# thomashirtz/samplers

Measured on AMD Instinct MI355X. Metric: posterior samples/sec (batch×steps/s), DPS CelebA-HQ-256 @1/2/4/8 GPU, higher is better.
Workload: dtype f32

## Files before the change

### include/samplers_hip.h

```cpp
#ifndef SAMPLERS_HIP_H
#define SAMPLERS_HIP_H

#include <stdint.h>

#ifdef __cplusplus
extern "C" {
#endif

typedef void* sp_stream_t;

enum {
    SP_OK = 0,
    SP_EINVAL = -1,
    SP_ELAUNCH = -2,
    SP_EUNSUPPORTED = -3
};

enum {
    SP_OP_IDENTITY = 0,
    SP_OP_INPAINT = 1,
    SP_OP_BLUR = 2,
    SP_OP_MASK = 3,
    SP_OP_SR = 4,
    SP_OP_PSF = 5,
// ... 157 lines not shown
                          int64_t batch, int64_t y_div, const sp_step_rec* sched,
                          const int32_t* cursor, float* v_out, float* rsq_partial,
                          sp_stream_t stream);
int sp_dps_residual_sched_ws(const sp_op* op, const float* x, const float* eps, const float* y,
                             int64_t batch, int64_t y_div, const sp_step_rec* sched,
                             const int32_t* cursor, float* v_out, float* rsq_partial,
                             float* work, sp_stream_t stream);
int sp_dps_update_sched(const sp_op* op, const float* x, const float* eps, const float* y,
                        const float* v, const float* w, const float* rsq_partial,
                        uint64_t seed, int64_t sample_offset, int64_t batch, int64_t y_div,
                        const sp_step_rec* sched, const int32_t* cursor, float* x_out,
                        sp_stream_t stream);

int sp_conv3x3_supported(int32_t cin, int32_t cout, int32_t height, int32_t width);
int64_t sp_conv3x3_packed_size(int32_t cin, int32_t cout);
int sp_conv3x3_pack(const float* w, int32_t cout, int32_t cin, int32_t input_vjp, float* wp,
                    sp_stream_t stream);
int sp_conv3x3_fwd(const float* x, const float* wp, const float* bias, int64_t n, int32_t cin,
                   int32_t cout, int32_t height, int32_t width, float* y, sp_stream_t stream);
int sp_conv3x3_bwd_input(const float* dy, const float* wp_vjp, int64_t n, int32_t cin,
                         int32_t cout, int32_t height, int32_t width, float* dx,
                         sp_stream_t stream);

int sp_conv3x3_thin_supported(int32_t cin, int32_t cout, int32_t height, int32_t width);
int sp_conv3x3_thin_fwd(const float* x, const float* w, const float* bias, int64_t n,
                        int32_t cin, int32_t cout, int32_t height, int32_t width, float* y,
                        sp_stream_t stream);
int sp_conv3x3_thin_bwd_input(const float* dy, const float* w, int64_t n, int32_t cin,
                              int32_t cout, int32_t height, int32_t width, float* dx,
                              sp_stream_t stream);

int sp_conv3x3_s2_supported(int32_t cin, int32_t cout, int32_t height, int32_t width,
                            int32_t input_vjp);
int sp_upsample2x_supported(int32_t height, int32_t width);
int sp_upsample2x(const float* x, int64_t planes, int32_t height, int32_t width, float* y,
                  sp_stream_t stream);
int sp_upsample2x_vjp(const float* dy, int64_t planes, int32_t height, int32_t width, float* dx,
                      sp_stream_t stream);
int sp_conv3x3_s2_pack(const float* w, int32_t cout, int32_t cin, int32_t input_vjp, float* wp,
                       sp_stream_t stream);
int sp_conv3x3_s2_fwd(const float* x, const float* wp, const float* bias, int64_t n, int32_t cin,
                      int32_t cout, int32_t height, int32_t width, float* y, sp_stream_t stream);
int sp_conv3x3_s2_bwd_input(const float* dy, const float* wp_vjp, int64_t n, int32_t cin,
                            int32_t cout, int32_t height, int32_t width, int32_t accumulate,
                            float* dx, sp_stream_t stream);
int64_t sp_conv3x3_s2_workspace(int64_t n, int32_t cin, int32_t cout, int32_t height, int32_t width,
                                int32_t input_vjp);
int sp_conv3x3_s2_fwd_ws(const float* x, const float* wp, const float* bias, int64_t n, int32_t cin,
                         int32_t cout, int32_t height, int32_t width, float* y, float* ws, int64_t ws_bytes,
                         sp_stream_t stream);
int sp_conv3x3_s2_bwd_input_ws(const float* dy, const float* wp_vjp, int64_t n, int32_t cin,
                               int32_t cout, int32_t height, int32_t width, int32_t accumulate,
                               float* dx, float* ws, int64_t ws_bytes, sp_stream_t stream);

int sp_wino3x3_supported(int32_t cin, int32_t cout, int32_t height, int32_t width);
int64_t sp_wino3x3_packed_size(int32_t cin, int32_t cout);
int sp_wino3x3_pack(const float* w, int32_t cout, int32_t cin, int32_t input_vjp, float* up,
                    sp_stream_t stream);
int sp_wino3x3_fwd(const float* x, const float* up, const float* bias, int64_t n, int32_t cin,
                   int32_t cout, int32_t height, int32_t width, float* y, sp_stream_t stream);
int sp_wino3x3_fwd_res(const float* x, const float* up, const float* bias, const float* res,
                       int64_t n, int32_t cin, int32_t cout, int32_t height, int32_t width,
                       float* y, sp_stream_t stream);
int sp_wino3x3_bwd_input(const float* dy, const float* up_vjp, int64_t n, int32_t cin,
                         int32_t cout, int32_t height, int32_t width, float* dx,
                         sp_stream_t stream);
int64_t sp_wino3x3_workspace(int64_t n, int32_t cin, int32_t cout, int32_t height, int32_t width);
int sp_wino3x3_fwd_ws(const float* x, const float* up, const float* bias, const float* res,
                      int64_t n, int32_t cin, int32_t cout, int32_t height, int32_t width,
                      float* y, float* ws, int64_t ws_bytes, sp_stream_t stream);
int sp_wino3x3_bwd_input_ws(const float* dy, const float* up_vjp, int64_t n, int32_t cin,
                            int32_t cout, int32_t height, int32_t width, float* dx, float* ws,
                            int64_t ws_bytes, sp_stream_t stream);
int sp_wino3x3_up_supported(int32_t cin, int32_t cout, int32_t height, int32_t width);
int sp_wino3x3_fwd_up(const float* x, const float* up, const float* bias, int64_t n, int32_t cin,
                      int32_t cout, int32_t height, int32_t width, float* y, sp_stream_t stream);
int sp_wino3x3_bwd_input_pool(const float* dy, const float* up_vjp, int64_t n, int32_t cin,
                              int32_t cout, int32_t height, int32_t width, float* dx,
                              sp_stream_t stream);

int sp_gemm_x6_supported(int32_t m, int32_t k, int64_t hw);
int64_t sp_gemm_x6_packed_size(int32_t m, int32_t k);
int sp_gemm_x6_pack(const float* w, int32_t m, int32_t k, int32_t trans, float* wp, sp_stream_t stream);
int sp_gemm_x6(const float* x1, int32_t c1, const float* x2, int32_t c2, const float* wp,
               const float* bias, const float* res, int64_t n, int64_t hw, float* y1, int32_t o1,
               float* y2, int32_t o2, sp_stream_t stream);

int sp_linear_x6_supported(int64_t tokens, int32_t k, int32_t m);
int sp_linear_x6(const float* x, const float* wp, const float* bias, const float* res, int64_t tokens,
                 int32_t k, int32_t m, float* y, sp_stream_t stream);

int sp_gemm_x6_layout_supported(int64_t n, int64_t hw, int32_t k, int32_t m);
int sp_gemm_x6_layout(const float* x, const float* wp, const float* bias, const float* res, int64_t n,
                      int64_t hw, int32_t k, int32_t m, int32_t in_tm, int32_t out_tm, float* y,
                      sp_stream_t stream);

int64_t sp_gemm_x6_workspace(int64_t n, int64_t hw, int32_t k, int32_t m);
int sp_gemm_x6_ws(const float* x1, int32_t c1, const float* x2, int32_t c2, const float* wp,
                  const float* bias, const float* res, int64_t n, int64_t hw, float* y1, int32_t o1,
                  float* y2, int32_t o2, float* ws, int64_t ws_bytes, sp_stream_t stream);
int sp_linear_x6_ws(const float* x, const float* wp, const float* bias, const float* res, int64_t tokens,
                    int32_t k, int32_t m, float* y, float* ws, int64_t ws_bytes, sp_stream_t stream);
int sp_gemm_x6_layout_ws(const float* x, const float* wp, const float* bias, const float* res, int64_t n,
                         int64_t hw, int32_t k, int32_t m, int32_t in_tm, int32_t out_tm, float* y, float* ws,
                         int64_t ws_bytes, sp_stream_t stream);

// ... 116 lines not shown
```

### samplers_amd/_hip.py

```python

from __future__ import annotations

import ctypes
import os
from pathlib import Path

import torch

LIB_PATH = Path(__file__).resolve().parent / "lib" / "libsamplers_hip.so"
DEBUG_LIB_PATH = Path(__file__).resolve().parent / "lib" / "debug" / "libsamplers_hip.so"

SP_OP_IDENTITY, SP_OP_INPAINT, SP_OP_BLUR, SP_OP_MASK, SP_OP_SR, SP_OP_PSF = 0, 1, 2, 3, 4, 5
SP_OP_PHASE = 6
HALO_KINDS = (SP_OP_BLUR, SP_OP_PSF)

_ERRORS = {-1: "invalid argument", -2: "kernel launch failed", -3: "unsupported"}


class HipLibraryError(RuntimeError):
    """The HIP library is missing, failed to load, or a call returned an error."""


class SpOp(ctypes.Structure):
    _fields_ = [
# ... 84 lines not shown
    "sp_adamw_step_until": (ctypes.c_int, [_P, _P, _P, _P, _I64, ctypes.POINTER(SpAdamWCoefs), _P,
                                           _P]),
    "sp_pixel_opt_step": (ctypes.c_int, [_OPP, _P, _P, _P, _P, _I64, _I64, _F,
                                         ctypes.POINTER(SpAdamWCoefs), _P, _P, _P]),
    "sp_opt_check": (ctypes.c_int, [_P, _I64, _F, ctypes.c_double, _P, _P, _P]),
    "sp_opt_check_plateau": (ctypes.c_int, [_P, _I64, _F, ctypes.c_double, _I64, _I64, _P, _P, _P,
                                            _P]),
    "sp_conv3x3_supported": (ctypes.c_int, [ctypes.c_int32] * 4),
    "sp_conv3x3_packed_size": (_I64, [ctypes.c_int32, ctypes.c_int32]),
    "sp_conv3x3_pack": (ctypes.c_int, [_P, ctypes.c_int32, ctypes.c_int32, ctypes.c_int32, _P, _P]),
    "sp_conv3x3_fwd": (ctypes.c_int, [_P, _P, _P, _I64, ctypes.c_int32, ctypes.c_int32,
                                      ctypes.c_int32, ctypes.c_int32, _P, _P]),
    "sp_conv3x3_bwd_input": (ctypes.c_int, [_P, _P, _I64, ctypes.c_int32, ctypes.c_int32,
                                            ctypes.c_int32, ctypes.c_int32, _P, _P]),
    "sp_conv3x3_thin_supported": (ctypes.c_int, [ctypes.c_int32] * 4),
    "sp_conv3x3_thin_fwd": (ctypes.c_int, [_P, _P, _P, _I64, ctypes.c_int32, ctypes.c_int32,
                                           ctypes.c_int32, ctypes.c_int32, _P, _P]),
    "sp_conv3x3_thin_bwd_input": (ctypes.c_int, [_P, _P, _I64, ctypes.c_int32, ctypes.c_int32,
                                                 ctypes.c_int32, ctypes.c_int32, _P, _P]),
    "sp_conv3x3_s2_supported": (ctypes.c_int, [ctypes.c_int32] * 5),
    "sp_upsample2x_supported": (ctypes.c_int, [ctypes.c_int32] * 2),
    "sp_upsample2x": (ctypes.c_int, [_P, _I64, ctypes.c_int32, ctypes.c_int32, _P, _P]),
    "sp_upsample2x_vjp": (ctypes.c_int, [_P, _I64, ctypes.c_int32, ctypes.c_int32, _P, _P]),
    "sp_attention_supported": (ctypes.c_int, [_I64, _I64, _I64, ctypes.c_int32]),
    "sp_attention_fwd": (ctypes.c_int, [_P, _P, _P, _I64, _I64, ctypes.c_int32, _F, _P, _P, _P]),
    "sp_attention_bwd": (ctypes.c_int, [_P, _P, _P, _P, _P, _P, _I64, _I64, ctypes.c_int32, _F,
                                        _P, _P, _P, _P, _P]),
    "sp_attention_mh_supported": (ctypes.c_int, [_I64, ctypes.c_int32, _I64, _I64, ctypes.c_int32]),
    "sp_attention6_supported": (ctypes.c_int, [_I64, ctypes.c_int32, _I64, ctypes.c_int32]),
    "sp_attention6_fwd_mh": (ctypes.c_int, [_P, _P, _P, _I64, ctypes.c_int32, _I64, ctypes.c_int32,
                                            ctypes.c_int32, ctypes.c_int32, _F, _P, _P, _P]),
    "sp_attention6_workspace": (_I64, [_I64, ctypes.c_int32, _I64, ctypes.c_int32]),
    "sp_attention6_fwd_ws": (ctypes.c_int, [_P, _P, _P, _I64, ctypes.c_int32, _I64, ctypes.c_int32,
                                            ctypes.c_int32, ctypes.c_int32, _F, _P, _P, _P, _I64, _P]),
    "sp_attention_bf16x6": (ctypes.c_int, [ctypes.c_int32]),
    "sp_attention_bf16x6_enabled": (ctypes.c_int, []),
    "sp_attention_fwd_mh": (ctypes.c_int, [_P, _P, _P, _I64, ctypes.c_int32, _I64, _I64, ctypes.c_int32,
                                           ctypes.c_int32, ctypes.c_int32, _I64, ctypes.c_int32, _F, _P, _P,
                                           _P]),
    "sp_attention_bwd_mh": (ctypes.c_int, [_P, _P, _P, _P, _P, _P, _I64, ctypes.c_int32, _I64, _I64,
                                           ctypes.c_int32, ctypes.c_int32, ctypes.c_int32, _I64,
                                           ctypes.c_int32, _F, _P, _P, _P, _P, _P]),
    "sp_conv3x3_s2_pack": (ctypes.c_int, [_P, ctypes.c_int32, ctypes.c_int32, ctypes.c_int32, _P, _P]),
    "sp_conv3x3_s2_fwd": (ctypes.c_int, [_P, _P, _P, _I64, ctypes.c_int32, ctypes.c_int32,
                                         ctypes.c_int32, ctypes.c_int32, _P, _P]),
    "sp_conv3x3_s2_bwd_input": (ctypes.c_int, [_P, _P, _I64, ctypes.c_int32, ctypes.c_int32,
                                               ctypes.c_int32, ctypes.c_int32, ctypes.c_int32, _P, _P]),
    "sp_conv3x3_s2_workspace": (_I64, [_I64, ctypes.c_int32, ctypes.c_int32, ctypes.c_int32, ctypes.c_int32,
                                       ctypes.c_int32]),
    "sp_conv3x3_s2_fwd_ws": (ctypes.c_int, [_P, _P, _P, _I64, ctypes.c_int32, ctypes.c_int32, ctypes.c_int32,
                                            ctypes.c_int32, _P, _P, _I64, _P]),
    "sp_conv3x3_s2_bwd_input_ws": (ctypes.c_int, [_P, _P, _I64, ctypes.c_int32, ctypes.c_int32, ctypes.c_int32,
                                                  ctypes.c_int32, ctypes.c_int32, _P, _P, _I64, _P]),
    "sp_wino3x3_supported": (ctypes.c_int, [ctypes.c_int32] * 4),
    "sp_gemm_x6_supported": (ctypes.c_int, [ctypes.c_int32, ctypes.c_int32, _I64]),
    "sp_gemm_x6_packed_size": (_I64, [ctypes.c_int32, ctypes.c_int32]),
    "sp_gemm_x6_pack": (ctypes.c_int, [_P, ctypes.c_int32, ctypes.c_int32, ctypes.c_int32, _P, _P]),
    "sp_gemm_x6": (ctypes.c_int, [_P, ctypes.c_int32, _P, ctypes.c_int32, _P, _P, _P, _I64, _I64,
                                  _P, ctypes.c_int32, _P, ctypes.c_int32, _P]),
    "sp_linear_x6_supported": (ctypes.c_int, [_I64, ctypes.c_int32, ctypes.c_int32]),
    "sp_linear_x6": (ctypes.c_int, [_P, _P, _P, _P, _I64, ctypes.c_int32, ctypes.c_int32, _P, _P]),
    "sp_gemm_x6_layout_supported": (ctypes.c_int, [_I64, _I64, ctypes.c_int32, ctypes.c_int32]),
    "sp_gemm_x6_layout": (ctypes.c_int, [_P, _P, _P, _P, _I64, _I64, ctypes.c_int32, ctypes.c_int32,
                                         ctypes.c_int32, ctypes.c_int32, _P, _P]),
    "sp_gemm_x6_workspace": (_I64, [_I64, _I64, ctypes.c_int32, ctypes.c_int32]),
    "sp_gemm_x6_ws": (ctypes.c_int, [_P, ctypes.c_int32, _P, ctypes.c_int32, _P, _P, _P, _I64, _I64,
                                     _P, ctypes.c_int32, _P, ctypes.c_int32, _P, _I64, _P]),
    "sp_linear_x6_ws": (ctypes.c_int, [_P, _P, _P, _P, _I64, ctypes.c_int32, ctypes.c_int32, _P, _P, _I64,
                                       _P]),
    "sp_gemm_x6_layout_ws": (ctypes.c_int, [_P, _P, _P, _P, _I64, _I64, ctypes.c_int32, ctypes.c_int32,
                                            ctypes.c_int32, ctypes.c_int32, _P, _P, _I64, _P]),
    "sp_layernorm_supported": (ctypes.c_int, [_I64, ctypes.c_int32]),
    "sp_layernorm_fwd": (ctypes.c_int, [_P, _P, _P, _I64, ctypes.c_int32, _F, _P, _P, _P, _P]),
    "sp_layernorm_bwd": (ctypes.c_int, [_P, _P, _P, _P, _P, _P, _I64, ctypes.c_int32, _P, _P]),
    "sp_geglu_fwd": (ctypes.c_int, [_P, _I64, ctypes.c_int32, _P, _P]),
    "sp_geglu_bwd": (ctypes.c_int, [_P, _P, _I64, ctypes.c_int32, _P, _P]),
    "sp_softmax_rows_supported": (ctypes.c_int, [_I64, ctypes.c_int32]),
    "sp_softmax_rows": (ctypes.c_int, [_P, _I64, ctypes.c_int32, _P, _P]),
    "sp_softmax_bwd_rows": (ctypes.c_int, [_P, _P, _I64, ctypes.c_int32, _F, _P]),
    "sp_conv1x1_small_supported": (ctypes.c_int, [ctypes.c_int32, ctypes.c_int32, _I64]),
    "sp_conv1x1_small": (ctypes.c_int, [_P, _P, _P, _I64, ctypes.c_int32, ctypes.c_int32, _I64,
                                        ctypes.c_int32, _P, _P]),
    "sp_wino3x3_packed_size": (_I64, [ctypes.c_int32, ctypes.c_int32]),
    "sp_wino3x3_pack": (ctypes.c_int, [_P, ctypes.c_int32, ctypes.c_int32, ctypes.c_int32, _P, _P]),
    "sp_wino3x3_fwd": (ctypes.c_int, [_P, _P, _P, _I64, ctypes.c_int32, ctypes.c_int32,
                                      ctypes.c_int32, ctypes.c_int32, _P, _P]),
    "sp_wino3x3_bwd_input": (ctypes.c_int, [_P, _P, _I64, ctypes.c_int32, ctypes.c_int32,
                                            ctypes.c_int32, ctypes.c_int32, _P, _P]),
    "sp_sched_timestep": (ctypes.c_int, [_P, _P, _P, _P]),
    "sp_sched_advance": (ctypes.c_int, [_P, _P]),
    "sp_dps_residual_sched": (ctypes.c_int, [_OPP, _P, _P, _P, _I64, _I64, _P, _P, _P, _P, _P]),
    "sp_dps_update_sched": (ctypes.c_int, [_OPP, _P, _P, _P, _P, _P, _P, _U64, _I64, _I64, _I64,
                                           _P, _P, _P, _P]),
    "sp_groupnorm_workspace": (_I64, [_I64, ctypes.c_int32, _I64, ctypes.c_int32]),
    "sp_groupnorm_silu_fwd": (ctypes.c_int, [_P, _P, _P, _P, _I64, ctypes.c_int32, _I64,
                                             ctypes.c_int32, _F, ctypes.c_int32, _P, _P, _P, _P,
                                             _P]),
    "sp_groupnorm_silu_bwd": (ctypes.c_int, [_P, _P, _P, _P, _P, _P, _P, _I64, ctypes.c_int32,
                                             _I64, ctypes.c_int32, ctypes.c_int32, _P, _P, _P]),
    "sp_groupnorm_silu_fwd2": (ctypes.c_int, [_P, _P, ctypes.c_int32, _P, _P, _P, _I64,
                                              ctypes.c_int32, _I64, ctypes.c_int32, _F,
                                              ctypes.c_int32, _P, _P, _P, _P, _P, _I64, _P]),
    "sp_groupnorm_silu_bwd2": (ctypes.c_int, [_P, _P, _P, ctypes.c_int32, _P, _P, _P, _P, _P,
                                              _I64, ctypes.c_int32, _I64, ctypes.c_int32,
                                              ctypes.c_int32, _P, _P, _P, _P, _P, _P, _P, _I64,
                                              _P]),
# ... 155 lines not shown
```

### samplers_amd/networks/layers.py

```python

from __future__ import annotations

import torch
import torch.nn.functional as F
from torch import Tensor, nn

from .. import _hip
from ..runtime import batch_invariant_enabled, split_k_enabled


def group_norm_act_torch(x: Tensor, groups: int, weight: Tensor | None, bias: Tensor | None,
                         eps: float, act: bool, chan_bias: Tensor | None = None) -> Tensor:
    if chan_bias is not None:
        x = x + chan_bias[:, :, None, None]
    y = F.group_norm(x, groups, weight, bias, eps)
    return F.silu(y) if act else y


_shape_cache: dict = {}


def _query(fn_name: str, *args: int) -> int:
    key = (fn_name, args)
    v = _shape_cache.get(key)
# ... 256 lines not shown
        return torch.nn.grad.conv2d_input(tuple(x_shape), module.weight, dy, padding=1)
    dx = torch.empty(tuple(x_shape), device=dy.device, dtype=torch.float32)
    if algo == "thin":
        _hip.check(lib.sp_conv3x3_thin_bwd_input(_hip.ptr(dy), _hip.ptr(module.weight.detach().contiguous()),
                                                 n, cin, cout, h, w, _hip.ptr(dx),
                                                 _hip.stream_of(dy)), "sp_conv3x3_thin_bwd_input")
        return dx
    if algo == "wino":
        ws = _wino_workspace(lib, n, cout, cin, h, w, dy.device)
        _hip.check(lib.sp_wino3x3_bwd_input_ws(_hip.ptr(dy), _hip.ptr(tile_pack(module, algo, True)),
                                               n, cin, cout, h, w, _hip.ptr(dx), _hip.ptr(ws),
                                               0 if ws is None else ws.numel() * 4,
                                               _hip.stream_of(dy)), "sp_wino3x3_bwd_input_ws")
        return dx
    _hip.check(lib.sp_conv3x3_bwd_input(_hip.ptr(dy), _hip.ptr(tile_pack(module, algo, True)), n, cin,
                                        cout, h, w, _hip.ptr(dx), _hip.stream_of(dy)),
               "sp_direct_conv3x3_bwd_input")
    return dx


class _Conv3x3Fn(torch.autograd.Function):
    @staticmethod
    def forward(ctx, x, weight, bias, module):
        ctx.module = module
        ctx.has_bias = bias is not None
        ctx.save_for_backward(x if weight.requires_grad else None, weight)
        ctx.x_shape = x.shape
        return conv3x3_forward(module, x)

    @staticmethod
    def backward(ctx, dy):
        x, weight = ctx.saved_tensors
        dx = dw = db = None
        if ctx.needs_input_grad[0]:
            dx = conv3x3_input_vjp(ctx.module, dy, ctx.x_shape)
        if ctx.needs_input_grad[1]:
            dw = torch.nn.grad.conv2d_weight(x, weight.shape, dy.contiguous(), padding=1)
        if ctx.has_bias and ctx.needs_input_grad[2]:
            db = dy.sum(dim=(0, 2, 3))
        return dx, dw, db, None


def tile_pack(module: nn.Conv2d, algo: str, input_vjp: bool) -> Tensor:
    w = module.weight
    key = (w.data_ptr(), w._version, w.device)
    cache = module.__dict__.setdefault("_tile_packs", {})
    if cache.get("key") != key:
        cache.clear()
        cache["key"] = key
    if (algo, input_vjp) not in cache:
        lib = _hip.load_library()
        cout, cin = w.shape[0], w.shape[1]
        wc = w.detach().contiguous()
        size_fn, fn = ((lib.sp_wino3x3_packed_size, lib.sp_wino3x3_pack) if algo == "wino"
                       else (lib.sp_conv3x3_packed_size, lib.sp_conv3x3_pack))
        out = torch.empty(int(size_fn(cin, cout)), device=w.device)
        _hip.check(fn(_hip.ptr(wc), cout, cin, int(input_vjp), _hip.ptr(out), _hip.stream_of(wc)),
                   f"sp_{algo}3x3_pack")
        cache[(algo, input_vjp)] = out
    return cache[(algo, input_vjp)]


class Conv3x3(nn.Conv2d):

    def __init__(self, cin: int, cout: int) -> None:
        super().__init__(cin, cout, 3, padding=1)

    def _pack(self, algo: str, input_vjp: bool) -> Tensor:
        return tile_pack(self, algo, input_vjp)

    def forward(self, x: Tensor) -> Tensor:
        if x.is_cuda and x.dtype == torch.bfloat16:
            from . import bf16
            if bf16.conv_supported(self, x):
                return bf16.conv3x3(self, x)
        if x.is_cuda and x.dtype == torch.float32 and x.dim() == 4:
            lib = _hip.load_library()
            n, cin, h, w = x.shape
            if _conv_algo(lib, cin, self.out_channels, h, w, conv_backend()) is not None:
                return _Conv3x3Fn.apply(x, self.weight, self.bias, self)
        miopen_fallback(x)
        return super().forward(x)



def _upsample2x_call(fn_name: str, src: Tensor, out_shape) -> Tensor:
    lib = _hip.load_library()
    n, c, h, w = (src.shape if fn_name == "sp_upsample2x" else out_shape)
    src = src.contiguous()
    out = torch.empty(tuple(out_shape), device=src.device, dtype=torch.float32)
    _hip.check(getattr(lib, fn_name)(_hip.ptr(src), n * c, h, w, _hip.ptr(out),
                                     _hip.stream_of(src)), fn_name)
    return out


class _Upsample2xFn(torch.autograd.Function):
    @staticmethod
    def forward(ctx, x):
        n, c, h, w = x.shape
        ctx.x_shape = x.shape
        return _upsample2x_call("sp_upsample2x", x, (n, c, 2 * h, 2 * w))

    @staticmethod
    def backward(ctx, dy):
        return _upsample2x_call("sp_upsample2x_vjp", dy, ctx.x_shape)


def _upconv_enabled() -> bool:
    import os

    return os.environ.get("SAMPLERS_AMD_UPCONV", "1").lower() not in ("0", "off", "false")
# ... 49 lines not shown
        return _UpsampleConv3x3Fn.apply(x, module.weight, module.bias, module)
    return module(upsample_nearest2x(x))


def upsample_nearest2x(x: Tensor) -> Tensor:
    if (x.is_cuda and x.dtype == torch.float32 and x.dim() == 4 and x.numel() > 0 and
            _hip.load_library().sp_upsample2x_supported(x.shape[2], x.shape[3])):
        return _Upsample2xFn.apply(x)
    return F.interpolate(x, scale_factor=2.0, mode="nearest")



def _s2_packed(module: nn.Conv2d, input_vjp: bool) -> Tensor:
    w = module.weight
    key = (w.data_ptr(), w._version, w.device)
    cache = module.__dict__.setdefault("_s2_packs", {})
    if cache.get("key") != key:
        cache.clear()
        cache["key"] = key
    if input_vjp not in cache:
        lib = _hip.load_library()
        cout, cin = w.shape[0], w.shape[1]
        wc = w.detach().contiguous()
        out = torch.empty(cin * cout * 9, device=w.device)
        _hip.check(lib.sp_conv3x3_s2_pack(_hip.ptr(wc), cout, cin, int(input_vjp), _hip.ptr(out),
                                          _hip.stream_of(wc)), "sp_conv3x3_s2_pack")
        cache[input_vjp] = out
    return cache[input_vjp]


def downsample_s2_supported(module: nn.Conv2d, x: Tensor) -> bool:
    if not (x.is_cuda and x.dtype == torch.float32 and x.dim() == 4) or conv_backend() == "miopen":
        return False
    lib = _hip.load_library()
    _, cin, h, w = x.shape
    cout = module.out_channels
    return bool(lib.sp_conv3x3_s2_supported(cin, cout, h, w, 0) and
                lib.sp_conv3x3_s2_supported(cin, cout, h, w, 1))


class SkipGrad:

    __slots__ = ("grad", "enabled")

    def __init__(self) -> None:
        self.grad: Tensor | None = None
        self.enabled = True

    def take(self) -> Tensor | None:
        g, self.grad = self.grad, None
        return g


def _s2_workspace(lib, n: int, cin: int, cout: int, h: int, w: int, vjp: int, device) -> tuple[Tensor | None, int]:
    nb = _query("sp_conv3x3_s2_workspace", n, cin, cout, h, w, vjp) if split_k_enabled() else 0
    if nb <= 0:
        return None, 0
    return torch.empty(nb // 4, device=device, dtype=torch.float32), nb


class _ConvS2Fn(torch.autograd.Function):
    @staticmethod
    def forward(ctx, x, weight, bias, module, box=None):
        lib = _hip.load_library()
        x = x.contiguous()
        n, cin, h, w = x.shape
        cout = module.out_channels
        y = torch.empty(n, cout, h // 2, w // 2, device=x.device, dtype=torch.float32)
        ws, nb = _s2_workspace(lib, n, cin, cout, h, w, 0, x.device)
        _hip.check(lib.sp_conv3x3_s2_fwd_ws(_hip.ptr(x), _hip.ptr(_s2_packed(module, False)),
                                            _hip.ptr(bias.contiguous()) if bias is not None else None,
                                            n, cin, cout, h, w, _hip.ptr(y), _hip.ptr(ws), nb, _hip.stream_of(x)),
                   "sp_conv3x3_s2_fwd")
        ctx.module = module
        ctx.box = box
        ctx.x_shape = x.shape
        return y

    @staticmethod
    def backward(ctx, dy):
        dx = None
        if ctx.needs_input_grad[0]:
            lib = _hip.load_library()
            n, cin, h, w = ctx.x_shape
            dx = ctx.box.take() if ctx.box is not None else None
            acc = dx is not None
            if dx is None:
                dx = torch.empty(tuple(ctx.x_shape), device=dy.device, dtype=torch.float32)
            ws, nb = _s2_workspace(lib, n, cin, ctx.module.out_channels, h, w, 1, dy.device)
            _hip.check(lib.sp_conv3x3_s2_bwd_input_ws(_hip.ptr(dy.contiguous()),
                                                      _hip.ptr(_s2_packed(ctx.module, True)),
                                                      n, cin, ctx.module.out_channels, h, w, int(acc),
                                                      _hip.ptr(dx), _hip.ptr(ws), nb, _hip.stream_of(dy)),
                       "sp_conv3x3_s2_bwd_input")
        return dx, None, None, None, None



def strided_full_supported(module: nn.Conv2d, x: Tensor) -> bool:
    if not (x.is_cuda and x.dtype == torch.float32 and x.dim() == 4) or module.weight.requires_grad:
        return False
    backend = conv_backend()
    if backend == "miopen":
        return False
    lib = _hip.load_library()
    _, cin, h, w = x.shape
    cout = module.out_channels
    fwd = _conv_algo(lib, cin, cout, h, w, backend)
    vjp = _conv_algo(lib, cout, cin, h, w, backend)
    ok = ("wino", "direct")
    return h % 2 == 0 and w % 2 == 0 and fwd in ok and vjp in ok


class _ConvS2FullFn(torch.autograd.Function):
    @staticmethod
    def forward(ctx, x, weight, bias, module, phase):
        y = conv3x3_forward(module, x.contiguous())
        ctx.module, ctx.phase, ctx.x_shape = module, phase, x.shape
        return y[:, :, phase::2, phase::2].contiguous()

    @staticmethod
    def backward(ctx, dy):
        dx = None
        if ctx.needs_input_grad[0]:
            n, _, h, w = ctx.x_shape
            dyf = dy.new_zeros((n, ctx.module.out_channels, h, w))
            dyf[:, :, ctx.phase::2, ctx.phase::2] = dy
            dx = conv3x3_input_vjp(ctx.module, dyf, ctx.x_shape)
        return dx, None, None, None, None


def conv3x3_stride2(module: nn.Conv2d, x: Tensor, padding: int) -> Tensor:
    if x.is_cuda and x.dtype == torch.bfloat16:
        from . import bf16
        if bf16.strided_supported(module, x):
            return bf16.conv3x3_stride2(module, x, padding)
    if strided_full_supported(module, x):
        return _ConvS2FullFn.apply(x, module.weight, module.bias, module, 0 if padding else 1)
    miopen_fallback(x)
    return module(x) if padding else module(F.pad(x, (0, 1, 0, 1)))


def downsample_conv(module: nn.Conv2d, x: Tensor, box: SkipGrad | None = None) -> Tensor:
    if x.is_cuda and x.dtype == torch.bfloat16:
        if box is not None:
            box.enabled = False
        return conv3x3_stride2(module, x, padding=0)
# ... 324 lines not shown
```

Measured before the change: 230.8.

## Add polyphase Winograd-style MFMA kernel for stride-2 3x3 conv fwd and input-VJP

Adds a new stride-2 3x3 convolution kernel that splits the stride-2 conv into polyphase components with a Winograd-like input transform. It runs the products on 32x32x2 f32 MFMA, using a software-pipelined 4-deep register ring and LDS staging for the forward path. The Python layer routes stride-2 conv forward and backward-input through it by default when supported and split-K workspace is not in use. It aims to cut the arithmetic and memory traffic of the existing direct stride-2 kernel. The cost is a new weight-packing format and a larger, more complex kernel that is harder to maintain.

```diff
diff --git a/include/samplers_hip.h b/include/samplers_hip.h
--- a/include/samplers_hip.h
+++ b/include/samplers_hip.h
@@ -233,6 +233,16 @@
 int sp_conv3x3_s2_bwd_input_ws(const float* dy, const float* wp_vjp, int64_t n, int32_t cin,
                                int32_t cout, int32_t height, int32_t width, int32_t accumulate,
                                float* dx, float* ws, int64_t ws_bytes, sp_stream_t stream);
+int sp_conv3x3_s2p_supported(int32_t cin, int32_t cout, int32_t height, int32_t width,
+                             int32_t input_vjp);
+int64_t sp_conv3x3_s2p_packed_size(int32_t cin, int32_t cout);
+int sp_conv3x3_s2p_pack(const float* w, int32_t cout, int32_t cin, int32_t input_vjp, float* up,
+                        sp_stream_t stream);
+int sp_conv3x3_s2p_fwd(const float* x, const float* up, const float* bias, int64_t n, int32_t cin,
+                       int32_t cout, int32_t height, int32_t width, float* y, sp_stream_t stream);
+int sp_conv3x3_s2p_bwd_input(const float* dy, const float* up_vjp, int64_t n, int32_t cin,
+                             int32_t cout, int32_t height, int32_t width, int32_t accumulate,
+                             float* dx, sp_stream_t stream);
 
 int sp_wino3x3_supported(int32_t cin, int32_t cout, int32_t height, int32_t width);
 int64_t sp_wino3x3_packed_size(int32_t cin, int32_t cout);
diff --git a/samplers_amd/_hip.py b/samplers_amd/_hip.py
--- a/samplers_amd/_hip.py
+++ b/samplers_amd/_hip.py
@@ -160,6 +160,13 @@
                                             ctypes.c_int32, _P, _P, _I64, _P]),
     "sp_conv3x3_s2_bwd_input_ws": (ctypes.c_int, [_P, _P, _I64, ctypes.c_int32, ctypes.c_int32, ctypes.c_int32,
                                                   ctypes.c_int32, ctypes.c_int32, _P, _P, _I64, _P]),
+    "sp_conv3x3_s2p_supported": (ctypes.c_int, [ctypes.c_int32] * 5),
+    "sp_conv3x3_s2p_packed_size": (_I64, [ctypes.c_int32, ctypes.c_int32]),
+    "sp_conv3x3_s2p_pack": (ctypes.c_int, [_P, ctypes.c_int32, ctypes.c_int32, ctypes.c_int32, _P, _P]),
+    "sp_conv3x3_s2p_fwd": (ctypes.c_int, [_P, _P, _P, _I64, ctypes.c_int32, ctypes.c_int32,
+                                          ctypes.c_int32, ctypes.c_int32, _P, _P]),
+    "sp_conv3x3_s2p_bwd_input": (ctypes.c_int, [_P, _P, _I64, ctypes.c_int32, ctypes.c_int32,
+                                                ctypes.c_int32, ctypes.c_int32, ctypes.c_int32, _P, _P]),
     "sp_wino3x3_supported": (ctypes.c_int, [ctypes.c_int32] * 4),
     "sp_gemm_x6_supported": (ctypes.c_int, [ctypes.c_int32, ctypes.c_int32, _I64]),
     "sp_gemm_x6_packed_size": (_I64, [ctypes.c_int32, ctypes.c_int32]),
diff --git a/samplers_amd/csrc/sp_conv_s2p.hip b/samplers_amd/csrc/sp_conv_s2p.hip
--- /dev/null
+++ b/samplers_amd/csrc/sp_conv_s2p.hip
@@ -0,0 +1,568 @@
+
+#define SP_TU 18
+#include "sp_common.h"
+
+namespace sp {
+
+typedef float p2_f32x16 __attribute__((ext_vector_type(16)));
+typedef float p2_f32x4 __attribute__((ext_vector_type(4)));
+typedef float p2_f32x2 __attribute__((ext_vector_type(2)));
+
+constexpr int P2_M = 64;
+constexpr int P2_OOB = 0x7FFFFFF0;
+constexpr int P2_USLOT = 16 * 64;
+
+struct P2Win { float a[3][3]; float b[2][3]; };
+struct P2U { p2_f32x4 u[4]; };
+
+struct P2Off { int v[8]; };
+
+template <bool VJP> struct P2Raw;
+template <> struct P2Raw<false> { p2_f32x4 a, b; float e; };
+template <> struct P2Raw<true> { p2_f32x2 r[3]; float e[3]; };
+
+template <int TSH> struct P2F {
+    static constexpr int TCW = 1 << TSH, TRW = 32 >> TSH, R = 4 * TRW + 1;
+    static constexpr int PS = TCW + 1, RS = 4 * PS, CS = R * RS;
+    static constexpr int PIECES = 2 * R * TCW;
+};
+constexpr int P2F_STAGE = 1344;
+constexpr int P2F_SINK = 2 * P2F_STAGE;
+constexpr int P2F_LDS = 3 * P2F_STAGE + 512;
+
+template <bool VJP, int S, int WV>
+__device__ __forceinline__ void p2_load(__amdgpu_buffer_rsrc_t rs, const P2Off& o, P2Raw<VJP>& w) {
+    if constexpr (!VJP) {
+        w.a = __builtin_bit_cast(p2_f32x4, __builtin_amdgcn_raw_buffer_load_b128(rs, o.v[0], 0, 0));
+        if constexpr (WV == 1)
+            w.b = __builtin_bit_cast(p2_f32x4, __builtin_amdgcn_raw_buffer_load_b128(rs, o.v[1], 0, 0));
+        if constexpr (WV == 2) w.e = __uint_as_float(__builtin_amdgcn_raw_buffer_load_b32(rs, o.v[2], 0, 0));
+    } else {
+#pragma unroll
+        for (int i = 0; i < 3; ++i)
+            w.r[i] = __builtin_bit_cast(p2_f32x2, __builtin_amdgcn_raw_buffer_load_b64(rs, o.v[i], 0, 0));
+#pragma unroll
+        for (int i = (S ? 1 : 0); i < 3; ++i)
+            w.e[i] = __uint_as_float(__builtin_amdgcn_raw_buffer_load_b32(rs, o.v[3 + i], 0, 0));
+    }
+}
+
+template <int TSH, int WV>
+__device__ __forceinline__ void p2f_stage(float* st, const P2Off& o, const P2Raw<false>& w) {
+    constexpr int PS = P2F<TSH>::PS;
+#pragma unroll
+    for (int q = 0; q < 4; ++q) st[o.v[3] + q * PS] = w.a[q];
+    if constexpr (WV == 1) {
+#pragma unroll
+        for (int q = 0; q < 4; ++q) st[o.v[4] + q * PS] = w.b[q];
+    }
+    if constexpr (WV == 2) st[o.v[5]] = w.e;
+}
+
+template <int S, int TSH>
+__device__ __forceinline__ void p2f_window(const float* st, int rd, P2Win& w) {
+    constexpr int PS = P2F<TSH>::PS, RS = P2F<TSH>::RS;
+    const float* p = st + rd;
+    if constexpr (S == 0) {
+#pragma unroll
+        for (int i = 0; i < 3; ++i)
+            w.a[i][0] = p[2 * i * RS], w.a[i][1] = p[2 * i * RS + 2 * PS], w.a[i][2] = p[2 * i * RS + 1];
+#pragma unroll
+        for (int i = 0; i < 2; ++i)
+            w.b[i][0] = p[(2 * i + 1) * RS + PS], w.b[i][1] = p[(2 * i + 1) * RS + 3 * PS];
+    } else {
+#pragma unroll
+        for (int i = 0; i < 3; ++i) w.a[i][0] = p[2 * i * RS + PS], w.a[i][1] = p[2 * i * RS + 3 * PS];
+#pragma unroll
+        for (int i = 0; i < 2; ++i)
+            w.b[i][0] = p[(2 * i + 1) * RS], w.b[i][1] = p[(2 * i + 1) * RS + 2 * PS],
+            w.b[i][2] = p[(2 * i + 1) * RS + 1];
+    }
+}
+
+template <int S>
+__device__ __forceinline__ void p2_window(const P2Raw<true>& x, P2Win& w) {
+    const auto& r = x.r;
+    const auto& e = x.e;
+    if constexpr (S == 0) {
+#pragma unroll
+        for (int i = 0; i < 3; ++i) w.a[i][0] = e[i], w.a[i][1] = r[i][0], w.a[i][2] = r[i][1];
+#pragma unroll
+        for (int i = 0; i < 2; ++i) w.b[i][0] = r[i + 1][0], w.b[i][1] = r[i + 1][1];
+    } else {
+#pragma unroll
+        for (int i = 0; i < 3; ++i) w.a[i][0] = r[i][0], w.a[i][1] = r[i][1];
+#pragma unroll
+        for (int i = 0; i < 2; ++i) w.b[i][0] = e[i + 1], w.b[i][1] = r[i + 1][0], w.b[i][2] = r[i + 1][1];
+    }
+}
+
+template <int S>
+__device__ __forceinline__ void p2_load_u(__amdgpu_buffer_rsrc_t urs, int lane, int soff, P2U& u) {
+#pragma unroll
+    for (int i = 0; i < 3; ++i)
+        u.u[i] = __builtin_bit_cast(p2_f32x4, __builtin_amdgcn_raw_buffer_load_b128(urs, (i * 64 + lane) * 16, soff, 0));
+    if constexpr (S == 0)
+        u.u[3][0] = __uint_as_float(__builtin_amdgcn_raw_buffer_load_b32(urs, (3 * 64 + lane) * 16, soff, 0));
+}
+
+template <int S>
+__device__ __forceinline__ void p2_transform(const P2Win& w, float (&v)[13]) {
+    if constexpr (S == 0) {
+        float t[3][3];
+#pragma unroll
+        for (int c = 0; c < 3; ++c) {
+            t[0][c] = w.a[0][c] - w.a[1][c];
+            t[1][c] = w.a[1][c];
+            t[2][c] = w.a[2][c] - w.a[1][c];
+        }
+#pragma unroll
+        for (int r = 0; r < 3; ++r) {
+            v[3 * r + 0] = t[r][0] - t[r][1];
+            v[3 * r + 1] = t[r][1];
+            v[3 * r + 2] = t[r][2] - t[r][1];
+        }
+#pragma unroll
+        for (int i = 0; i < 4; ++i) v[9 + i] = w.b[i >> 1][i & 1];
+    } else {
+#pragma unroll
+        for (int c = 0; c < 2; ++c) {
+            v[0 + c] = w.a[0][c] - w.a[1][c];
+            v[2 + c] = w.a[1][c];
+            v[4 + c] = w.a[2][c] - w.a[1][c];
+        }
+#pragma unroll
+        for (int r = 0; r < 2; ++r) {
+            v[6 + 3 * r + 0] = w.b[r][0] - w.b[r][1];
+            v[6 + 3 * r + 1] = w.b[r][1];
+            v[6 + 3 * r + 2] = w.b[r][2] - w.b[r][1];
+        }
+        v[12] = 0.f;
+    }
+}
+
+template <bool VJP> struct P2Ring {
+    P2Raw<VJP> xs[4];
+    P2U us[4];
+    float v[2][13];
+};
+
+#define P2_MFMA(j)                                                                                        \
+    if constexpr ((j) < (S ? 12 : 13)) {                                                                  \
+        acc[j] = __builtin_amdgcn_mfma_f32_32x32x2f32(u.u[(j) >> 2][(j) & 3], vc[j], acc[j], 0, 0, 0);    \
+        __builtin_amdgcn_sched_barrier(0);                                                                \
+    }                                                                                                     \
+    static_assert(true, "")
+#define P2_WALL                    \
+    asm volatile("" ::: "memory"); \
+    __builtin_amdgcn_sched_barrier(0)
+
+template <int S, int U>
+__device__ __forceinline__ void p2_step(const float* __restrict__ inn, int64_t iplane2, int ibytes,
+                                        const P2Off& o, __amdgpu_buffer_rsrc_t urs, int lane, int ustride,
+                                        int q, int nk, P2Ring<true>& r, p2_f32x16 (&acc)[13]) {
+    asm volatile("" : "+s"(q));
+    const P2U& u = r.us[U];
+    const float(&vc)[13] = r.v[U & 1];
+    const int qn = min(q + 3, nk - 1);
+    P2_MFMA(0);
+    {
+        const auto rs = __builtin_amdgcn_make_buffer_rsrc(const_cast<float*>(inn + qn * iplane2), (short)0,
+                                                          ibytes, 0x00020000);
+        p2_load<true, S, S>(rs, o, r.xs[(U + 3) & 3]);
+    }
+    P2_WALL;
+    P2_MFMA(1);
+    p2_load_u<S>(urs, lane, qn * ustride, r.us[(U + 3) & 3]);
+    P2_WALL;
+    P2_MFMA(2);
+    P2_MFMA(3);
+    P2_MFMA(4);
+    P2_MFMA(5);
+    P2_MFMA(6);
+    {
+        P2Win w;
+        p2_window<S>(r.xs[(U + 1) & 3], w);
+        p2_transform<S>(w, r.v[(U + 1) & 1]);
+    }
+    P2_WALL;
+    P2_MFMA(7);
+    P2_MFMA(8);
+    P2_MFMA(9);
+    P2_MFMA(10);
+    P2_MFMA(11);
+    P2_MFMA(12);
+}
+
+template <int WV, int TSH, int U>
+__device__ __forceinline__ void p2f_step(const float* __restrict__ inn, int64_t iplane2, int ibytes,
+                                         const P2Off& o, __amdgpu_buffer_rsrc_t urs, int lane, int ustride,
+                                         int q, int nk, float* xl, P2Ring<false>& r, p2_f32x16 (&acc)[13]) {
+    constexpr int S = WV & 1;
+    asm volatile("" : "+s"(q));
+    const P2U& u = r.us[U];
+    const float(&vc)[13] = r.v[U & 1];
+    P2_MFMA(0);
+    {
+        const auto rs = __builtin_amdgcn_make_buffer_rsrc(
+            const_cast<float*>(inn + min(q + 4, nk - 1) * iplane2), (short)0, ibytes, 0x00020000);
+        p2_load<false, S, WV>(rs, o, r.xs[U]);
+    }
+    P2_WALL;
+    P2_MFMA(1);
+    p2_load_u<S>(urs, lane, min(q + 3, nk - 1) * ustride, r.us[(U + 3) & 3]);
+    P2_WALL;
+    P2_MFMA(2);
+    p2f_stage<TSH, WV>(xl + (U & 1) * P2F_STAGE, o, r.xs[(U + 2) & 3]);
+    P2_WALL;
+    P2_MFMA(3);
+    P2_MFMA(4);
+    P2Win w;
+    p2f_window<S, TSH>(xl + ((U + 1) & 1) * P2F_STAGE, o.v[6], w);
+    P2_WALL;
+    P2_MFMA(5);
+    P2_MFMA(6);
+    P2_MFMA(7);
+    p2_transform<S>(w, r.v[(U + 1) & 1]);
+    P2_WALL;
+    P2_MFMA(8);
+    P2_MFMA(9);
+    P2_MFMA(10);
+    P2_MFMA(11);
+    P2_MFMA(12);
+    __builtin_amdgcn_s_waitcnt(0xc07f);
+    __builtin_amdgcn_s_barrier();
+    P2_WALL;
+}
+#undef P2_MFMA
+#undef P2_WALL
+
+template <bool VJP, int WV, int TSH>
+__device__ __forceinline__ void p2_body(const float* __restrict__ in, const float* __restrict__ up,
+                                        const float* __restrict__ bias, float* __restrict__ out,
+                                        int K, int M, int H, int W, int acc_in, float* ex, float* xl) {
+    constexpr int S = WV & 1;
+    const int Ho = H / 2, Wo = W / 2, TH = Ho / 2, TW = Wo / 2;
+    constexpr int tsh = TSH, tcw = 1 << tsh, trw = 32 >> tsh;
+    const int mblocks = M / P2_M;
+    const int mb = blockIdx.x % mblocks, grp = blockIdx.x / mblocks;
+    const int gw = TW / tcw, per_img = gw * (TH / trw);
+    const int n = grp / per_img, g = grp - n * per_img;
+    const int tid = threadIdx.x, lane = tid & 63, hh = lane >> 5, l = lane & 31;
+    const int wv = __builtin_amdgcn_readfirstlane(tid >> 6);
+    const int ti = (g / gw) * trw + (l >> tsh), tj = (g % gw) * tcw + (l & (tcw - 1));
+    const int m0 = mb * P2_M + (wv >> 1) * 32;
+    SP_DCHECK(TW % tcw == 0 && TH % trw == 0 && ti < TH && tj < TW && m0 + 32 <= M && K % 8 == 0);
+
+    const int ih = VJP ? Ho : H, iw = VJP ? Wo : W;
+    const int64_t iplane = (int64_t)ih * iw;
+    const float* inn = in + (int64_t)n * K * iplane;
+    const int hoff = hh * static_cast<int>(iplane);
+    P2Off o;
+    if constexpr (!VJP) {
+        using F = P2F<TSH>;
+        const int r0 = 4 * (g / gw) * trw, c0 = 4 * (g % gw) * tcw;
+        const int plane = static_cast<int>(iplane);
+#pragma unroll
+        for (int j = 0; j < 2; ++j) {
+            const int it = j ? kBlock + lane : tid;
+            const int c = it / (F::R * tcw), rem = it - c * (F::R * tcw), row = rem >> tsh, c4 = rem & (tcw - 1);
+            const bool have = it < F::PIECES;
+            SP_DCHECK(!have || (c < 2 && row < F::R && c0 + 4 * c4 + 3 < W));
+            o.v[j] = have && r0 + row < H ? (c * plane + (r0 + row) * W + c0 + 4 * c4) * 4 : P2_OOB;
+            o.v[3 + j] = have ? c * F::CS + row * F::RS + c4 : P2F_SINK + tid;
+        }
+        {
+            const int c = lane / F::R, row = lane - c * F::R;
+            const bool have = lane < 2 * F::R;
+            o.v[2] = have && r0 + row < H && c0 + 4 * tcw < W ? (c * plane + (r0 + row) * W + c0 + 4 * tcw) * 4
+                                                              : P2_OOB;
+            o.v[5] = have ? c * F::CS + row * F::RS + tcw : P2F_SINK + tid;
+        }
+        o.v[6] = hh * F::CS + 4 * (l >> tsh) * F::RS + (l & (tcw - 1));
+        static_assert(2 * F::CS <= P2F_STAGE && P2F_SINK + kBlock + 3 * F::PS <= 2 * P2F_STAGE + 512, "LDS stage");
+    } else {
+#pragma unroll
+        for (int i = 0; i < 3; ++i) {
+            const int r = 2 * ti - 1 + i;
+            o.v[i] = r >= 0 ? (hoff + r * Wo + 2 * tj) * 4 : P2_OOB;
+            o.v[3 + i] = (r >= 0 && tj > 0) ? (hoff + r * Wo + 2 * tj - 1) * 4 : P2_OOB;
+        }
+    }
+    const int nk = K / 2;
+    const int ibytes = static_cast<int>(2 * iplane * 4);
+    const int ustride = (M / 32) * 2 * P2_USLOT * 4;
+    const auto urs = __builtin_amdgcn_make_buffer_rsrc(
+        const_cast<float*>(up + ((int64_t)(m0 / 32) * 2 + S) * P2_USLOT), (short)0, 0x7FFFFFFF, 0x00020000);
+
+    p2_f32x16 acc[13];
+#pragma unroll
+    for (int j = 0; j < 13; ++j) acc[j] = p2_f32x16{};
+    P2Ring<VJP> ring;
+    const int64_t iplane2 = 2 * iplane;
+    auto in_rs = [&](int q) {
+        return __builtin_amdgcn_make_buffer_rsrc(const_cast<float*>(inn + q * iplane2), (short)0, ibytes, 0x00020000);
+    };
+#define P2_WALL                    \
+    asm volatile("" ::: "memory"); \
+    __builtin_amdgcn_sched_barrier(0)
+    if constexpr (VJP) {
+#pragma unroll
+        for (int q = 0; q < 3; ++q) {
+            p2_load<VJP, S, WV>(in_rs(q), o, ring.xs[q]);
+            P2_WALL;
+            p2_load_u<S>(urs, lane, q * ustride, ring.us[q]);
+            P2_WALL;
+        }
+        P2Win w;
+        p2_window<S>(ring.xs[0], w);
+        p2_transform<S>(w, ring.v[0]);
+        for (int ks = 0; ks < nk; ks += 4) {
+            p2_step<S, 0>(inn, iplane2, ibytes, o, urs, lane, ustride, ks, nk, ring, acc);
+            p2_step<S, 1>(inn, iplane2, ibytes, o, urs, lane, ustride, ks + 1, nk, ring, acc);
+            p2_step<S, 2>(inn, iplane2, ibytes, o, urs, lane, ustride, ks + 2, nk, ring, acc);
+            p2_step<S, 3>(inn, iplane2, ibytes, o, urs, lane, ustride, ks + 3, nk, ring, acc);
+        }
+    } else {
+        p2_load<VJP, S, WV>(in_rs(0), o, ring.xs[0]);
+        P2_WALL;
+#pragma unroll
+        for (int q = 0; q < 3; ++q) {
+            p2_load<VJP, S, WV>(in_rs(q + 1), o, ring.xs[q + 1]);
+            P2_WALL;
+            p2_load_u<S>(urs, lane, q * ustride, ring.us[q]);
+            P2_WALL;
+        }
+        p2f_stage<TSH, WV>(xl, o, ring.xs[0]);
+        p2f_stage<TSH, WV>(xl + P2F_STAGE, o, ring.xs[1]);
+        __builtin_amdgcn_s_waitcnt(0xc07f);
+        __builtin_amdgcn_s_barrier();
+        P2_WALL;
+        {
+            P2Win w;
+            p2f_window<S, TSH>(xl, o.v[6], w);
+            p2_transform<S>(w, ring.v[0]);
+        }
+        P2_WALL;
+        __builtin_amdgcn_s_waitcnt(0xc07f);
+        __builtin_amdgcn_s_barrier();
+        P2_WALL;
+        for (int ks = 0; ks < nk; ks += 4) {
+            p2f_step<WV, TSH, 0>(inn, iplane2, ibytes, o, urs, lane, ustride, ks, nk, xl, ring, acc);
+            p2f_step<WV, TSH, 1>(inn, iplane2, ibytes, o, urs, lane, ustride, ks + 1, nk, xl, ring, acc);
+            p2f_step<WV, TSH, 2>(inn, iplane2, ibytes, o, urs, lane, ustride, ks + 2, nk, xl, ring, acc);
+            p2f_step<WV, TSH, 3>(inn, iplane2, ibytes, o, urs, lane, ustride, ks + 3, nk, xl, ring, acc);
+        }
+    }
+#undef P2_WALL
+
+    float* exw = ex + wv * (VJP ? 16 * 64 * 4 : 16 * 64 * 2);
+    float* exp_ = ex + (wv ^ 1) * (VJP ? 16 * 64 * 4 : 16 * 64 * 2);
+    if constexpr (!VJP) {
+        p2_f32x2 keep[16];
+#pragma unroll
+        for (int e = 0; e < 16; ++e) {
+            float y[2][2];
+            if constexpr (S == 0) {
+                float t[2][3];
+#pragma unroll
+                for (int r = 0; r < 2; ++r)
+#pragma unroll
+                    for (int c = 0; c < 3; ++c) t[r][c] = acc[3 * r + c][e] + acc[3 * r + 3 + c][e];
+#pragma unroll
+                for (int r = 0; r < 2; ++r)
+#pragma unroll
+                    for (int c = 0; c < 2; ++c) y[r][c] = (t[r][c] + t[r][c + 1]) + acc[9 + 2 * r + c][e];
+            } else {
+#pragma unroll
+                for (int r = 0; r < 2; ++r)
+#pragma unroll
+                    for (int c = 0; c < 2; ++c)
+                        y[r][c] = (acc[2 * r + c][e] + acc[2 * r + 2 + c][e]) +
+                                  (acc[6 + 3 * r + c][e] + acc[6 + 3 * r + c + 1][e]);
+            }
+            keep[e] = p2_f32x2{y[S][0], y[S][1]};
+            *reinterpret_cast<p2_f32x2*>(&exw[(e * 64 + lane) * 2]) = p2_f32x2{y[1 - S][0], y[1 - S][1]};
+        }
+        __syncthreads();
+        float* on = out + (int64_t)n * M * Ho * Wo;
+#pragma unroll
+        for (int e = 0; e < 16; ++e) {
+            const int m = m0 + (e & 3) + 8 * (e >> 2) + 4 * hh;
+            const p2_f32x2 other = *reinterpret_cast<const p2_f32x2*>(&exp_[(e * 64 + lane) * 2]);
+            p2_f32x2 v = keep[e] + other;
+            if (bias) v += bias[m];
+            *reinterpret_cast<p2_f32x2*>(on + ((int64_t)m * Ho + 2 * ti + S) * Wo + 2 * tj) = v;
+        }
+    } else {
+        float* dn = out + (int64_t)n * M * H * W;
+        p2_f32x4 prev[16][2];
+#pragma unroll
+        for (int e = 0; e < 16; ++e) {
+            const int m = m0 + (e & 3) + 8 * (e >> 2) + 4 * hh;
+#pragma unroll
+            for (int r = 0; r < 2; ++r)
+                prev[e][r] = acc_in ? *reinterpret_cast<const p2_f32x4*>(
+                                          dn + ((int64_t)m * H + 4 * ti + 2 * r + S) * W + 4 * tj)
+                                    : p2_f32x4{};
+        }
+        asm volatile("" ::: "memory");
+        __builtin_amdgcn_sched_barrier(0);
+        p2_f32x4 keep[16];
+#pragma unroll
+        for (int e = 0; e < 16; ++e) {
+            float pa[2][2], pb[2][2];
+            if constexpr (S == 0) {
+                float t[2][3];
+#pragma unroll
+                for (int r = 0; r < 2; ++r)
+#pragma unroll
+                    for (int c = 0; c < 3; ++c) t[r][c] = acc[3 * r + c][e] + acc[3 * r + 3 + c][e];
+#pragma unroll
+                for (int r = 0; r < 2; ++r)
+#pragma unroll
+                    for (int c = 0; c < 2; ++c) pa[r][c] = t[r][c] + t[r][c + 1], pb[r][c] = acc[9 + 2 * r + c][e];
+            } else {
+#pragma unroll
+                for (int r = 0; r < 2; ++r)
+#pragma unroll
+                    for (int c = 0; c < 2; ++c) {
+                        pb[r][c] = acc[2 * r + c][e] + acc[2 * r + 2 + c][e];
+                        pa[r][c] = acc[6 + 3 * r + c][e] + acc[6 + 3 * r + c + 1][e];
+                    }
+            }
+            keep[e] = p2_f32x4{pa[0][0], pa[0][1], pa[1][0], pa[1][1]};
+            *reinterpret_cast<p2_f32x4*>(&exw[(e * 64 + lane) * 4]) = p2_f32x4{pb[0][0], pb[0][1], pb[1][0], pb[1][1]};
+        }
+        __syncthreads();
+#pragma unroll
+        for (int e = 0; e < 16; ++e) {
+            const int m = m0 + (e & 3) + 8 * (e >> 2) + 4 * hh;
+            const p2_f32x4 other = *reinterpret_cast<const p2_f32x4*>(&exp_[(e * 64 + lane) * 4]);
+#pragma unroll
+            for (int r = 0; r < 2; ++r) {
+                p2_f32x4* d = reinterpret_cast<p2_f32x4*>(dn + ((int64_t)m * H + 4 * ti + 2 * r + S) * W + 4 * tj);
+                p2_f32x4 v{keep[e][2 * r], other[2 * r], keep[e][2 * r + 1], other[2 * r + 1]};
+                if (acc_in) v = prev[e][r] + v;
+                *d = v;
+            }
+        }
+    }
+}
+
+template <bool VJP, int TSH>
+__global__ __launch_bounds__(kBlock, 1) void k_s2p(const float* __restrict__ in, const float* __restrict__ up,
+                                                   const float* __restrict__ bias, float* __restrict__ out,
+                                                   int K, int M, int H, int W, int acc_in) {
+    __shared__ __attribute__((aligned(16))) float ex[4 * 16 * 64 * (VJP ? 4 : 2)];
+    __shared__ __attribute__((aligned(16))) float xl[VJP ? 4 : P2F_LDS];
+    const int wv = threadIdx.x >> 6;
+    if constexpr (VJP) {
+        if (wv & 1)
+            p2_body<VJP, 1, TSH>(in, up, bias, out, K, M, H, W, acc_in, ex, xl);
+        else
+            p2_body<VJP, 0, TSH>(in, up, bias, out, K, M, H, W, acc_in, ex, xl);
+    } else {
+        if (wv == 0)
+            p2_body<VJP, 0, TSH>(in, up, bias, out, K, M, H, W, acc_in, ex, xl);
+        else if (wv == 1)
+            p2_body<VJP, 1, TSH>(in, up, bias, out, K, M, H, W, acc_in, ex, xl);
+        else if (wv == 2)
+            p2_body<VJP, 2, TSH>(in, up, bias, out, K, M, H, W, acc_in, ex, xl);
+        else
+            p2_body<VJP, 3, TSH>(in, up, bias, out, K, M, H, W, acc_in, ex, xl);
+    }
+}
+
+__global__ void k_s2p_pack(const float* __restrict__ w, int cout, int cin, int vjp, float* __restrict__ up) {
+    const int M = vjp ? cin : cout, K = vjp ? cout : cin;
+    const int64_t total = (int64_t)M * K * 32;
+    const int64_t i = (int64_t)blockIdx.x * blockDim.x + threadIdx.x;
+    if (i >= total) return;
+    const int e = static_cast<int>(i & 3), lane = static_cast<int>((i >> 2) & 63), piece = static_cast<int>((i >> 8) & 3);
+    const int s = static_cast<int>((i >> 10) & 1);
+    const int64_t rest = i >> 11;
+    const int mb = static_cast<int>(rest % (M / 32)), ks = static_cast<int>(rest / (M / 32));
+    const int j = piece * 4 + e, m = mb * 32 + (lane & 31), k = 2 * ks + (lane >> 5);
+    int tr, tc;
+    if (s == 0) {
+        if (j < 9) tr = j / 3, tc = j % 3;
+        else if (j < 13) tr = 3, tc = 3;
+        else { up[i] = 0.f; return; }
+    } else {
+        if (j < 6) tr = j / 2, tc = 3;
+        else if (j < 12) tr = 3, tc = (j - 6) % 3;
+        else { up[i] = 0.f; return; }
+    }
+    const int t0 = vjp ? 2 : 0, t1 = 2 - t0;
+    auto mask = [&](int t) { return t == 3 ? 2 : t == 0 ? (1 << t0) : t == 2 ? (1 << t1) : 5; };
+    const int rm = mask(tr), cm = mask(tc);
+    const int co = vjp ? k : m, ci = vjp ? m : k;
+    const float* g = w + ((int64_t)co * cin + ci) * 9;
+    double sum = 0.0;
+    for (int a = 0; a < 3; ++a)
+        for (int b = 0; b < 3; ++b)
+            if ((rm >> a & 1) && (cm >> b & 1)) sum += static_cast<double>(g[a * 3 + b]);
+    up[i] = static_cast<float>(sum);
+}
+
+}
+
+using namespace sp;
+
+static int s2p_tsh(int32_t width) { return (width / 4) % 32 == 0 ? 5 : 4; }
+
+extern "C" {
+
+int sp_conv3x3_s2p_supported(int32_t cin, int32_t cout, int32_t height, int32_t width, int32_t input_vjp) {
+    if (cin <= 0 || cout <= 0 || height <= 0 || width <= 0 || height % 8 || width % 64) return 0;
+    const int m = input_vjp ? cin : cout, k = input_vjp ? cout : cin;
+    return m % P2_M == 0 && k % 8 == 0 && (int64_t)height * width < (int64_t(1) << 27);
+}
+
+int64_t sp_conv3x3_s2p_packed_size(int32_t cin, int32_t cout) { return (int64_t)cin * cout * 32; }
+
+int sp_conv3x3_s2p_pack(const float* w, int32_t cout, int32_t cin, int32_t input_vjp, float* up,
+                        sp_stream_t stream) {
+    if (!w || !up || cout <= 0 || cin <= 0) return SP_EINVAL;
+    const int m = input_vjp ? cin : cout, k = input_vjp ? cout : cin;
+    if (m % 32 || k % 2) return SP_EINVAL;
+    const int64_t total = (int64_t)cin * cout * 32;
+    launch(0, k_s2p_pack, dim3(static_cast<unsigned>((total + 255) / 256)), dim3(256),
+           static_cast<hipStream_t>(stream), w, cout, cin, input_vjp ? 1 : 0, up);
+    return check_launch("sp_conv3x3_s2p_pack");
+}
+
+static int s2p_launch(int vjp, const float* in, const float* up, const float* bias, int64_t n, int32_t cin,
+                      int32_t cout, int32_t height, int32_t width, int32_t accumulate, float* out,
+                      sp_stream_t stream) {
+    if (!sp_conv3x3_s2p_supported(cin, cout, height, width, vjp) || n < 0) return SP_EINVAL;
+    if (n == 0) return SP_OK;
+    if (!in || !up || !out) return SP_EINVAL;
+    const int m = vjp ? cin : cout, k = vjp ? cout : cin;
+    const int64_t groups = n * (height / 4) * (int64_t)(width / 4) / 32 * (m / P2_M);
+    if (groups >= (int64_t(1) << 31) || (int64_t)cin * cout * 32 * 4 >= (int64_t(1) << 31)) return SP_EINVAL;
+    const double flops = 12.5 * n * cin * cout * (height / 2) * (width / 2);
+    hipStream_t s = static_cast<hipStream_t>(stream);
+    const dim3 grid(static_cast<unsigned>(groups)), block(kBlock);
+    const bool wide = s2p_tsh(width) == 5;
+    if (!vjp)
+        launch_w(TK_CONV3X3_FWD, flops, wide ? k_s2p<false, 5> : k_s2p<false, 4>, grid, block, s, in, up, bias, out,
+                 k, m, height, width, 0);
+    else
+        launch_w(TK_CONV3X3_BWD_INPUT, flops, wide ? k_s2p<true, 5> : k_s2p<true, 4>, grid, block, s, in, up, bias,
+                 out, k, m, height, width, accumulate ? 1 : 0);
+    return check_launch(vjp ? "sp_conv3x3_s2p_bwd_input" : "sp_conv3x3_s2p_fwd");
+}
+
+int sp_conv3x3_s2p_fwd(const float* x, const float* up, const float* bias, int64_t n, int32_t cin,
+                       int32_t cout, int32_t height, int32_t width, float* y, sp_stream_t stream) {
+    return s2p_launch(0, x, up, bias, n, cin, cout, height, width, 0, y, stream);
+}
+
+int sp_conv3x3_s2p_bwd_input(const float* dy, const float* up_vjp, int64_t n, int32_t cin, int32_t cout,
+                             int32_t height, int32_t width, int32_t accumulate, float* dx, sp_stream_t stream) {
+    return s2p_launch(1, dy, up_vjp, nullptr, n, cin, cout, height, width, accumulate, dx, stream);
+}
+
+}
diff --git a/samplers_amd/networks/layers.py b/samplers_amd/networks/layers.py
--- a/samplers_amd/networks/layers.py
+++ b/samplers_amd/networks/layers.py
@@ -332,11 +332,11 @@
         lib = _hip.load_library()
         cout, cin = w.shape[0], w.shape[1]
         wc = w.detach().contiguous()
-        size_fn, fn = ((lib.sp_wino3x3_packed_size, lib.sp_wino3x3_pack) if algo == "wino"
-                       else (lib.sp_conv3x3_packed_size, lib.sp_conv3x3_pack))
+        stem = {"wino": "sp_wino3x3", "direct": "sp_conv3x3", "s2p": "sp_conv3x3_s2p"}[algo]
+        size_fn, fn = getattr(lib, stem + "_packed_size"), getattr(lib, stem + "_pack")
         out = torch.empty(int(size_fn(cin, cout)), device=w.device)
         _hip.check(fn(_hip.ptr(wc), cout, cin, int(input_vjp), _hip.ptr(out), _hip.stream_of(wc)),
-                   f"sp_{algo}3x3_pack")
+                   stem + "_pack")
         cache[(algo, input_vjp)] = out
     return cache[(algo, input_vjp)]
 
@@ -492,6 +492,17 @@
         return g
 
 
+def s2_backend() -> str:
+    import os
+
+    return os.environ.get("SAMPLERS_AMD_S2", "polyphase").lower()
+
+
+def _s2_polyphase(cin: int, cout: int, h: int, w: int, vjp: int, split_bytes: int) -> bool:
+    return (split_bytes <= 0 and s2_backend() != "direct" and
+            bool(_query("sp_conv3x3_s2p_supported", cin, cout, h, w, vjp)))
+
+
 def _s2_workspace(lib, n: int, cin: int, cout: int, h: int, w: int, vjp: int, device) -> tuple[Tensor | None, int]:
     nb = _query("sp_conv3x3_s2_workspace", n, cin, cout, h, w, vjp) if split_k_enabled() else 0
     if nb <= 0:
@@ -508,10 +519,17 @@
         cout = module.out_channels
         y = torch.empty(n, cout, h // 2, w // 2, device=x.device, dtype=torch.float32)
         ws, nb = _s2_workspace(lib, n, cin, cout, h, w, 0, x.device)
-        _hip.check(lib.sp_conv3x3_s2_fwd_ws(_hip.ptr(x), _hip.ptr(_s2_packed(module, False)),
-                                            _hip.ptr(bias.contiguous()) if bias is not None else None,
-                                            n, cin, cout, h, w, _hip.ptr(y), _hip.ptr(ws), nb, _hip.stream_of(x)),
-                   "sp_conv3x3_s2_fwd")
+        if _s2_polyphase(cin, cout, h, w, 0, nb):
+            _hip.check(lib.sp_conv3x3_s2p_fwd(_hip.ptr(x), _hip.ptr(tile_pack(module, "s2p", False)),
+                                              _hip.ptr(bias.contiguous()) if bias is not None else None,
+                                              n, cin, cout, h, w, _hip.ptr(y), _hip.stream_of(x)),
+                       "sp_conv3x3_s2p_fwd")
+        else:
+            _hip.check(lib.sp_conv3x3_s2_fwd_ws(_hip.ptr(x), _hip.ptr(_s2_packed(module, False)),
+                                                _hip.ptr(bias.contiguous()) if bias is not None else None,
+                                                n, cin, cout, h, w, _hip.ptr(y), _hip.ptr(ws), nb,
+                                                _hip.stream_of(x)),
+                       "sp_conv3x3_s2_fwd")
         ctx.module = module
         ctx.box = box
         ctx.x_shape = x.shape
@@ -527,12 +545,20 @@
             acc = dx is not None
             if dx is None:
                 dx = torch.empty(tuple(ctx.x_shape), device=dy.device, dtype=torch.float32)
-            ws, nb = _s2_workspace(lib, n, cin, ctx.module.out_channels, h, w, 1, dy.device)
-            _hip.check(lib.sp_conv3x3_s2_bwd_input_ws(_hip.ptr(dy.contiguous()),
-                                                      _hip.ptr(_s2_packed(ctx.module, True)),
-                                                      n, cin, ctx.module.out_channels, h, w, int(acc),
-                                                      _hip.ptr(dx), _hip.ptr(ws), nb, _hip.stream_of(dy)),
-                       "sp_conv3x3_s2_bwd_input")
+            cout = ctx.module.out_channels
+            ws, nb = _s2_workspace(lib, n, cin, cout, h, w, 1, dy.device)
+            if _s2_polyphase(cin, cout, h, w, 1, nb):
+                _hip.check(lib.sp_conv3x3_s2p_bwd_input(_hip.ptr(dy.contiguous()),
+                                                        _hip.ptr(tile_pack(ctx.module, "s2p", True)),
+                                                        n, cin, cout, h, w, int(acc), _hip.ptr(dx),
+                                                        _hip.stream_of(dy)),
+                           "sp_conv3x3_s2p_bwd_input")
+            else:
+                _hip.check(lib.sp_conv3x3_s2_bwd_input_ws(_hip.ptr(dy.contiguous()),
+                                                          _hip.ptr(_s2_packed(ctx.module, True)),
+                                                          n, cin, cout, h, w, int(acc),
+                                                          _hip.ptr(dx), _hip.ptr(ws), nb, _hip.stream_of(dy)),
+                           "sp_conv3x3_s2_bwd_input")
         return dx, None, None, None, None
 
 
```

After: 232.4 (median of 6 runs). About the same (+0.7%).
